# xmlyqing00/V-FloodNet

Hardware: AMD Instinct MI355X
Metric: segmented frames/sec at 480p (higher is better)
Workload: dtype f32

## Files before the change

v-floodnet_amd/csrc/memory_read.hip:

```cpp
#include "common.h"
#include "../../include/vfn_hip.h"
#include <type_traits>
#include <cstdlib>

namespace {

constexpr int DK = 128, DV = 512;
constexpr int CH = 64;

__device__ __forceinline__ int swz(int row, int chunk) { return row * DK + ((chunk ^ (row & 15)) << 2); }

__device__ __forceinline__ int swz64(int row, int chunk) { return row * CH + ((chunk ^ (row & 15)) << 2); }

struct ChunkRegs { f32x4 v[8]; };
__device__ __forceinline__ void chunk_load(ChunkRegs& R, const float* src, int valid, int tid) {
    const int c = tid & 31;
#pragma unroll
    for (int j = 0; j < 8; ++j) {
        const int r = (tid >> 5) + 8 * j;
        const int rr = r < valid ? r : 0;
        R.v[j] = *reinterpret_cast<const f32x4*>(src + (size_t)rr * DK + c * 4);
        if (r >= valid) R.v[j] = f32x4{0.f, 0.f, 0.f, 0.f};
    }
}
// ... 64 lines not shown
        const __bf16 x = (__bf16)a[e], y = (__bf16)b[e];
        h[e] = x; h[4 + e] = y;
        l[e] = (__bf16)(a[e] - (float)x); l[4 + e] = (__bf16)(b[e] - (float)y);
    }
}
__device__ __forceinline__ int swzk(int row, int half, int chunk) { return row * 512 + half * 256 + ((chunk ^ (row & 15)) << 4); }
__device__ __forceinline__ int swzq(int row, int chunk) { return row * 256 + ((chunk ^ (row & 15)) << 4); }

template <int NT, bool X3>
__device__ __forceinline__ void convert_chunk_inplace(float* sK, int tid) {
    constexpr int TPR = NT / CH;
    constexpr int F4 = 32 / TPR;
    const int r = tid / TPR, part = tid % TPR;
    f32x4 v[F4];
#pragma unroll
    for (int j = 0; j < F4; ++j) v[j] = *reinterpret_cast<const f32x4*>(sK + swz(r, part * F4 + j));
    __syncthreads();
    char* base = reinterpret_cast<char*>(sK);
#pragma unroll
    for (int j = 0; j < F4; j += 2) {
        bf16x8 h, l;
        split8(v[j], v[j + 1], h, l);
        const int chunk = (part * F4 + j) >> 1;
        *reinterpret_cast<bf16x8*>(base + swzk(r, 0, chunk)) = h;
        if constexpr (X3) *reinterpret_cast<bf16x8*>(base + swzk(r, 1, chunk)) = l;
    }
    __syncthreads();
}

template <bool X3>
__device__ __forceinline__ void mfma_lp(f32x16& acc, const bf16x8& ah, const bf16x8& al, const bf16x8& bh, const bf16x8& bl) {
    if constexpr (X3) {
        acc = __builtin_amdgcn_mfma_f32_32x32x16_bf16(al, bh, acc, 0, 0, 0);
        acc = __builtin_amdgcn_mfma_f32_32x32x16_bf16(ah, bl, acc, 0, 0, 0);
    }
    acc = __builtin_amdgcn_mfma_f32_32x32x16_bf16(ah, bh, acc, 0, 0, 0);
}

__device__ __forceinline__ float fast_exp(float x) { return __expf(x); }

__device__ __forceinline__ void chunk_range(int B, int nsplit, int split, int& c_lo, int& c_hi) {
    const int nchunks = (B + CH - 1) / CH;
    const int per = (nchunks + nsplit - 1) / nsplit;
    c_lo = split * per;
    c_hi = min(nchunks, c_lo + per);
}

constexpr int QTS = 128;

#ifdef VFN_CENSUS
__device__ unsigned long long vfn_census_buf[4096 * 4];
#endif

struct scan_gather { const int* list; const int* count; };

template <int MODE, int PREC = 0, bool GATHER = false>
__global__ __launch_bounds__(256, 2)
void bank_scan_kernel(const vfn_bankscan_desc p, const scan_gather gather) {
#ifdef VFN_CENSUS
    const unsigned long long census_t0 = __builtin_amdgcn_s_memrealtime();
#endif
    extern __shared__ __attribute__((aligned(16))) char smem[];
    float* sKb = reinterpret_cast<float*>(smem);
    __shared__ int s_item;

    const int tid = threadIdx.x, lane = tid & 63, wave = tid >> 6;
    const int li = lane & 31, lh = lane >> 5;
    const int qtiles = (p.HW + QTS - 1) / QTS;
    int total = p.nsplit * qtiles * p.obj_n;
    if constexpr (GATHER) {
        total = 0;
        for (int o = 0; o < p.obj_n; ++o) total += p.nsplit * ((gather.count[o] + QTS - 1) / QTS);
    }
  for (;;) {
    if (tid == 0) s_item = atomicAdd(p.work_counter, 1);
    __syncthreads();
    int item = s_item;
    __syncthreads();
    if (item >= total) break;
    int obj, qt, split;
    if constexpr (GATHER) {
        obj = 0;
        for (;;) {
            const int n = p.nsplit * ((gather.count[obj] + QTS - 1) / QTS);
            if (item < n) break;
            item -= n; ++obj;
        }
        const int qtl = (gather.count[obj] + QTS - 1) / QTS;
        qt = item % qtl;
        split = item / qtl;
    } else {
        obj = item % p.obj_n;
        qt = (item / p.obj_n) % qtiles;
        split = item / (p.obj_n * qtiles);
    }
    const int q0 = qt * QTS + wave * 32;
    const int ncol = GATHER ? gather.count[obj] : p.HW;
    const int B = p.bank_len[obj];
    const bool lp_image = PREC != 0 && p.bank_k_lp != nullptr;
    const float* K = (lp_image ? reinterpret_cast<const float*>(p.bank_k_lp) : p.bank_k) + (size_t)obj * p.stride_k;
    const float* Q = p.q + (size_t)(p.q_per_obj ? obj : 0) * p.stride_q;

    int c_lo, c_hi;
    chunk_range(B, p.nsplit, split, c_lo, c_hi);
    if (c_lo < c_hi) chunk_load_async(sKb, K + (size_t)c_lo * CH * DK, min(CH, B - c_lo * CH), wave, lane);

    f32x4 qf[PREC == 0 ? 16 : 1];
    bf16x8 qh[PREC == 0 ? 1 : 8], ql[PREC == 2 ? 8 : 1];
    {
        int q = min(q0 + li, ncol - 1);
        if constexpr (GATHER) q = gather.list[(size_t)obj * p.HW + q];
        if constexpr (PREC == 0) {
            const float* qrow = Q + (size_t)q * p.ldq + 4 * lh;
#pragma unroll
            for (int kk = 0; kk < 16; ++kk) qf[kk] = *reinterpret_cast<const f32x4*>(qrow + 8 * kk);
        } else {
            const float* qrow = Q + (size_t)q * p.ldq + 8 * lh;
#pragma unroll
            for (int g = 0; g < 8; ++g) {
                const f32x4 x0 = *reinterpret_cast<const f32x4*>(qrow + 16 * g);
                const f32x4 x1 = *reinterpret_cast<const f32x4*>(qrow + 16 * g + 4);
                if constexpr (PREC == 2) split8(x0, x1, qh[g], ql[g]);
                else qh[g] = cvt8(x0, x1);
            }
        }
    }

    float run_m = -INFINITY, run_l = 0.f;
    int run_i = 0x7fffffff;
    float run_2 = -INFINITY;
    bool sick = false;
    __syncthreads();

    for (int c = c_lo; c < c_hi; ++c) {
        const int b0 = c * CH;
        const float* sK = sKb + ((c - c_lo) & 1) * CH * DK;
#ifndef VFN_ABLATE_KLOAD
        if (c + 1 < c_hi)
            chunk_load_async(sKb + ((c + 1 - c_lo) & 1) * CH * DK, K + (size_t)(b0 + CH) * DK, min(CH, B - b0 - CH), wave, lane);
#endif
        f32x4 scv[MODE >= 1 ? 2 : 1][MODE >= 1 ? 4 : 1];
        float rs_lane = 1.f;
        if constexpr (MODE >= 1) {
            const float* rs = p.rowscale + (size_t)obj * p.stride_rs;
#pragma unroll
            for (int i = 0; i < 2; ++i)
#pragma unroll
                for (int g = 0; g < 4; ++g) scv[i][g] = *reinterpret_cast<const f32x4*>(rs + b0 + 32 * i + 4 * lh + 8 * g);
            if constexpr (MODE == 2) rs_lane = rs[b0 + lane];
        }
// ... 116 lines not shown
                }
            if constexpr (MODE == 2) sick |= (b0 + lane < B) && !(rs_lane > 0.f && rs_lane < 1e12f);
        }
        __syncthreads();
    }

    {
        const float om = __shfl_xor(run_m, 32, 64);
        if (MODE == 0) {
            const float ol = __shfl_xor(run_l, 32, 64);
            const float mn = fmaxf(run_m, om);
            float l = 0.f;
            if (mn > -INFINITY) l = run_l * expf(run_m - mn) + ol * expf(om - mn);
            run_m = mn; run_l = l;
        } else {
            const int oi = __shfl_xor(run_i, 32, 64);
            if constexpr (MODE == 2) {
                const float o2 = __shfl_xor(run_2, 32, 64);
                if (om > run_m || (om == run_m && oi < run_i)) run_2 = fmaxf(run_m, o2);
                else run_2 = fmaxf(run_2, om);
            }
            if (om > run_m || (om == run_m && oi < run_i)) { run_m = om; run_i = oi; }
        }
    }
    if constexpr (MODE == 2) {
        if (__ballot(sick) != 0) run_2 = INFINITY;
    }
#ifdef VFN_CENSUS
    if (threadIdx.x == 0) {
        const int lin = blockIdx.y * gridDim.x + blockIdx.x;
        if (lin < 4096) {
            unsigned hw_id, xcc;
            asm volatile("s_getreg_b32 %0, hwreg(HW_REG_HW_ID)" : "=s"(hw_id));
            asm volatile("s_getreg_b32 %0, hwreg(HW_REG_XCC_ID)" : "=s"(xcc));
            vfn_census_buf[lin * 4] = census_t0; vfn_census_buf[lin * 4 + 1] = __builtin_amdgcn_s_memrealtime();
            vfn_census_buf[lin * 4 + 2] = hw_id; vfn_census_buf[lin * 4 + 3] = xcc;
        }
    }
#endif
    const int q = q0 + li;
    if (lh == 0 && q < ncol) {
        if constexpr (MODE == 2) {
            float* dst = p.part + (((size_t)obj * p.nsplit + split) * p.HW + q) * 4;
            *reinterpret_cast<f32x4*>(dst) = f32x4{run_m, __int_as_float(run_i), run_2, 0.f};
        } else {
            float* dst = p.part + (((size_t)obj * p.nsplit + split) * p.HW + q) * 2;
            dst[0] = run_m;
            dst[1] = (MODE == 0) ? run_l : __int_as_float(run_i);
        }
    }
  }
}

constexpr size_t SCAN_PIPE_LDS = 2 * (size_t)CH * DK * 2 + 2 * CH * sizeof(float);
constexpr unsigned SCAN_PIPE_SC0 = 2 * CH * DK * 2;

template <int MODE>
__global__ __launch_bounds__(256, 2)
void bank_scan_pipe_kernel(const vfn_bankscan_desc p) {
    extern __shared__ __attribute__((aligned(16))) char smem[];
    __shared__ int s_item;

    const int tid = threadIdx.x, lane = tid & 63, wave = tid >> 6;
    const int li = lane & 31, lh = lane >> 5;
    const int qtiles = (p.HW + QTS - 1) / QTS;
    const int total = p.nsplit * qtiles * p.obj_n;
    const int krow = tid >> 2, kc4 = (tid & 3) * 4;
    const unsigned klane_off = (unsigned)krow * 512u + (unsigned)kc4 * 16u;
  for (;;) {
    if (tid == 0) s_item = atomicAdd(p.work_counter, 1);
    __syncthreads();
    const int item = s_item;
    __syncthreads();
    if (item >= total) break;
    const int obj = item % p.obj_n;
    const int qt = (item / p.obj_n) % qtiles;
    const int split = item / (p.obj_n * qtiles);
    const int q0 = qt * QTS + wave * 32;
    const int B = p.bank_len[obj];
    const char* Kimg = reinterpret_cast<const char*>(p.bank_k_lp) + (size_t)obj * p.stride_k * 4;
    const float* Q = p.q + (size_t)(p.q_per_obj ? obj : 0) * p.stride_q;

    int c_lo, c_hi;
    chunk_range(B, p.nsplit, split, c_lo, c_hi);

    u32x4 kst[2][4];
    f32x4 sst[2];
    const float* rs = MODE == 1 ? p.rowscale + (size_t)obj * p.stride_rs : nullptr;
    auto load_k = [&](int c, auto SET_) {
        constexpr int set = decltype(SET_)::value;
        const int b0 = c * CH;
        const __amdgpu_buffer_rsrc_t r = __builtin_amdgcn_make_buffer_rsrc(const_cast<char*>(Kimg + (size_t)b0 * 512), 0, min(CH, B - b0) * 512, 0x00020000);
#pragma unroll
        for (int j = 0; j < 4; ++j) kst[set][j] = __builtin_amdgcn_raw_buffer_load_b128(r, klane_off, 16 * j, 0);
        if constexpr (MODE == 1) { if (tid < 16) sst[set] = *reinterpret_cast<const f32x4*>(rs + b0 + 4 * tid); }
    };
    auto store_k = [&](int buf, auto SET_) {
        constexpr int set = decltype(SET_)::value;
        char* d = smem + buf * (CH * DK * 2);
#pragma unroll
        for (int j = 0; j < 4; ++j) *reinterpret_cast<u32x4*>(d + swzq(krow, kc4 + j)) = kst[set][j];
        if constexpr (MODE == 1) { if (tid < 16) *reinterpret_cast<f32x4*>(smem + SCAN_PIPE_SC0 + buf * (CH * 4) + tid * 16) = sst[set]; }
    };
    using Z0 = std::integral_constant<int, 0>; using Z1 = std::integral_constant<int, 1>;
    if (c_lo < c_hi) load_k(c_lo, Z0{});
    if (c_lo + 1 < c_hi) load_k(c_lo + 1, Z1{});

    bf16x8 qh[8];
    {
        const int q = min(q0 + li, p.HW - 1);
        const float* qrow = Q + (size_t)q * p.ldq + 8 * lh;
#pragma unroll
        for (int g = 0; g < 8; ++g) {
            const f32x4 x0 = *reinterpret_cast<const f32x4*>(qrow + 16 * g);
            const f32x4 x1 = *reinterpret_cast<const f32x4*>(qrow + 16 * g + 4);
            qh[g] = cvt8(x0, x1);
        }
    }

    float run_m = -INFINITY, run_l = 0.f;
    int run_i = 0x7fffffff;
    if (c_lo < c_hi) store_k(0, Z0{});
    __syncthreads();

    auto body = [&](auto PAR_, int c) {
        constexpr int PAR = decltype(PAR_)::value;
        const int b0 = c * CH;
        const char* kb = smem + PAR * (CH * DK * 2);
        if (c + 2 < c_hi) load_k(c + 2, PAR_);
        f32x4 scv[MODE == 1 ? 2 : 1][MODE == 1 ? 4 : 1];
        if constexpr (MODE == 1) {
            const float* sS = reinterpret_cast<const float*>(smem + SCAN_PIPE_SC0 + PAR * (CH * 4));
#pragma unroll
            for (int i = 0; i < 2; ++i)
#pragma unroll
                for (int g = 0; g < 4; ++g) scv[i][g] = *reinterpret_cast<const f32x4*>(sS + 32 * i + 4 * lh + 8 * g);
        }
        f32x16 acc[2];
#pragma unroll
        for (int i = 0; i < 2; ++i)
#pragma unroll
            for (int r = 0; r < 16; ++r) acc[i][r] = 0.f;
#pragma unroll
        for (int g = 0; g < 8; ++g) {
#pragma unroll
            for (int i = 0; i < 2; ++i) {
                const bf16x8 ah = *reinterpret_cast<const bf16x8*>(kb + swzq(32 * i + li, 2 * g + lh));
                acc[i] = __builtin_amdgcn_mfma_f32_32x32x16_bf16(ah, qh[g], acc[i], 0, 0, 0);
            }
        }
        if (MODE == 0) {
            if (b0 + CH <= B) {
                float mx = acc[0][0];
#pragma unroll
                for (int i = 0; i < 2; ++i)
#pragma unroll
                    for (int r = 0; r < 16; ++r) mx = fmaxf(mx, acc[i][r]);
                const float mn = fmaxf(run_m, mx * p.scale);
                float sum = 0.f;
#pragma unroll
                for (int i = 0; i < 2; ++i)
#pragma unroll
                    for (int r = 0; r < 16; ++r) sum += fast_exp(acc[i][r] * p.scale - mn);
                run_l = run_l * expf(run_m - mn) + sum;
                run_m = mn;
            } else {
                float mx = -INFINITY;
#pragma unroll
                for (int i = 0; i < 2; ++i)
#pragma unroll
                    for (int r = 0; r < 16; ++r) {
                        const int row = b0 + 32 * i + 4 * lh + (r & 3) + 8 * (r >> 2);
                        const float s_ = acc[i][r] * p.scale;
                        acc[i][r] = s_;
                        if (row < B) mx = fmaxf(mx, s_);
                    }
                const float mn = fmaxf(run_m, mx);
                if (mn > -INFINITY) {
                    float sum = 0.f;
#pragma unroll
                    for (int i = 0; i < 2; ++i)
#pragma unroll
                        for (int r = 0; r < 16; ++r) {
                            const int row = b0 + 32 * i + 4 * lh + (r & 3) + 8 * (r >> 2);
                            if (row < B) sum += fast_exp(acc[i][r] - mn);
                        }
                    run_l = run_l * expf(run_m - mn) + sum;
                    run_m = mn;
                }
            }
        } else {
#pragma unroll
            for (int i = 0; i < 2; ++i)
#pragma unroll
                for (int g = 0; g < 4; ++g) {
                    const int row0 = b0 + 32 * i + 4 * lh + 8 * g;
                    const f32x4 sc = scv[MODE == 1 ? i : 0][MODE == 1 ? g : 0];
#pragma unroll
                    for (int j = 0; j < 4; ++j) {
                        const int row = row0 + j;
                        if (row < B) {
                            const float s_ = acc[i][4 * g + j] * sc[j];
                            if (s_ > run_m) { run_m = s_; run_i = row; }
                        }
                    }
                }
        }
        if (c + 1 < c_hi) store_k(PAR ^ 1, std::integral_constant<int, PAR ^ 1>{});
        __syncthreads();
    };
    for (int c = c_lo; c < c_hi; c += 2) {
        body(std::integral_constant<int, 0>{}, c);
        if (c + 1 < c_hi) body(std::integral_constant<int, 1>{}, c + 1);
    }

    {
        const float om = __shfl_xor(run_m, 32, 64);
        if (MODE == 0) {
            const float ol = __shfl_xor(run_l, 32, 64);
            const float mn = fmaxf(run_m, om);
            float l = 0.f;
            if (mn > -INFINITY) l = run_l * expf(run_m - mn) + ol * expf(om - mn);
            run_m = mn; run_l = l;
        } else {
            const int oi = __shfl_xor(run_i, 32, 64);
            if (om > run_m || (om == run_m && oi < run_i)) { run_m = om; run_i = oi; }
        }
    }
    const int q = q0 + li;
    if (lh == 0 && q < p.HW) {
        float* dst = p.part + (((size_t)obj * p.nsplit + split) * p.HW + q) * 2;
        dst[0] = run_m;
        dst[1] = (MODE == 0) ? run_l : __int_as_float(run_i);
    }
  }
}

template <int MODE>
__global__ void bank_scan_finish_kernel(const float* __restrict__ part, int nsplit, int HW, int obj_n,
                                        float* __restrict__ ml, int* __restrict__ idx, float* __restrict__ corr,
                                        const float* __restrict__ colscale) {
    const int t = blockIdx.x * blockDim.x + threadIdx.x;
    const int i = min(t >> 3, obj_n * HW - 1), j = t & 7;
    const bool live = (t >> 3) < obj_n * HW;
    const int obj = i / HW, q = i - obj * HW;
    float m = -INFINITY, x = (MODE == 0) ? 0.f : __int_as_float(0x7fffffff);
    auto fold = [&](float om, float ox) {
        if (MODE == 0) {
            const float mn = fmaxf(m, om);
            if (mn > -INFINITY) x = x * expf(m - mn) + ox * expf(om - mn);
            m = mn;
        } else {
            const int i0 = __float_as_int(x), i1 = __float_as_int(ox);
            if (om > m || (om == m && i1 < i0)) { m = om; x = ox; }
        }
    };
    for (int s = j; s < nsplit; s += 8) {
        const float* src = part + (((size_t)obj * nsplit + s) * HW + q) * 2;
        fold(src[0], src[1]);
    }
    const int base = (threadIdx.x & 63) & ~7;
#pragma unroll
    for (int o = 1; o < 8; ++o) {
        const float om = __shfl(m, base + o, 64), ox = __shfl(x, base + o, 64);
        if (j == 0) fold(om, ox);
    }
    if (j != 0 || !live) return;
    if (MODE == 0) { ml[(size_t)i * 2] = m; ml[(size_t)i * 2 + 1] = x; }
    else { idx[i] = __float_as_int(x); corr[i] = m * colscale[i]; }
}

constexpr float MATCH_EPS_REL = 1.25e-4f;
constexpr float MATCH_EPS_ABS = 5.421010862427522e-20f;
constexpr float MATCH_QNORM_MAX = 1.152921504606846976e18f;

__global__ __launch_bounds__(64)
void bank_match_certify_kernel(const vfn_bankmatch_desc p) {
    const int lane = threadIdx.x, li = lane & 31, lh = lane >> 5;
    const int obj = blockIdx.y, q0 = blockIdx.x * 32;
    const int q = q0 + li, qc = min(q, p.HW - 1);
    float m = -INFINITY, m2 = -INFINITY;
    int bi = 0x7fffffff;
    auto fold = [&](float om, int oi, float o2) {
        if (om > m || (om == m && oi < bi)) { m2 = fmaxf(fmaxf(m, m2), o2); m = om; bi = oi; }
        else m2 = fmaxf(fmaxf(m2, om), o2);
    };
    const float* part = p.part_x3 + ((size_t)obj * p.nsplit * p.HW + qc) * 4;
#pragma unroll 4
    for (int s = lh; s < p.nsplit; s += 2) {
        const f32x4 v = *reinterpret_cast<const f32x4*>(part + (size_t)s * p.HW * 4);
        fold(v[0], __float_as_int(v[1]), v[2]);
    }
    fold(__shfl_xor(m, 32, 64), __shfl_xor(bi, 32, 64), __shfl_xor(m2, 32, 64));

    const size_t col = (size_t)obj * p.HW + qc;
    const float qn = p.qnorm[col];
    const float margin = 4.f * (MATCH_EPS_REL * qn + MATCH_EPS_ABS);
    const bool cert = q < p.HW && qn > 0.f && qn <= MATCH_QNORM_MAX && m > -INFINITY && m < INFINITY && (m - m2) > margin;

    const float* krow = p.bank_k + (size_t)obj * p.stride_k + (size_t)(cert ? bi : 0) * DK + 4 * lh;
    const float* qrow = p.q + (size_t)obj * p.stride_q + (size_t)qc * p.ldq + 4 * lh;
    f32x16 acc;
#pragma unroll
    for (int r = 0; r < 16; ++r) acc[r] = 0.f;
#pragma unroll
    for (int kk = 0; kk < 16; ++kk) {
        f32x4 a = *reinterpret_cast<const f32x4*>(krow + 8 * kk);
        const f32x4 b = *reinterpret_cast<const f32x4*>(qrow + 8 * kk);
        if (!cert) a = f32x4{0.f, 0.f, 0.f, 0.f};
#pragma unroll
        for (int t = 0; t < 4; ++t) acc = __builtin_amdgcn_mfma_f32_32x32x2f32(a[t], b[t], acc, 0, 0, 0);
    }
    const int rsel = (li & 3) + 4 * (li >> 3);
    float dot = 0.f;
#pragma unroll
    for (int r = 0; r < 16; ++r) dot = (r == rsel) ? acc[r] : dot;
    if (lh != ((li >> 2) & 1)) return;
    if (cert) {
        const float s_ = dot * p.rowscale[(size_t)obj * p.stride_rs + bi];
        p.match_idx[col] = bi;
        p.match_corr[col] = s_ * p.colscale[col];
    } else if (q < p.HW) {
        const int pos = atomicAdd(p.ucount + obj, 1);
        p.ulist[(size_t)obj * p.HW + pos] = q;
        if (p.utotal) atomicAdd(p.utotal + obj, 1);
    }
}

__global__ void bank_match_finish_listed_kernel(const float* __restrict__ part, int nsplit, int HW, int obj_n,
                                                const int* __restrict__ ulist, const int* __restrict__ ucount,
                                                int* __restrict__ idx, float* __restrict__ corr, const float* __restrict__ colscale) {
    const int t = blockIdx.x * blockDim.x + threadIdx.x;
    const int i = min(t >> 3, obj_n * HW - 1), j = t & 7;
    const int obj = i / HW, pos = i - obj * HW;
    const bool live = (t >> 3) < obj_n * HW && pos < ucount[obj];
    float m = -INFINITY, x = __int_as_float(0x7fffffff);
    auto fold = [&](float om, float ox) {
        const int i0 = __float_as_int(x), i1 = __float_as_int(ox);
        if (om > m || (om == m && i1 < i0)) { m = om; x = ox; }
    };
    if (live)
        for (int s = j; s < nsplit; s += 8) {
            const float* src = part + (((size_t)obj * nsplit + s) * HW + pos) * 2;
            fold(src[0], src[1]);
        }
    const int base = (threadIdx.x & 63) & ~7;
#pragma unroll
    for (int o = 1; o < 8; ++o) {
        const float om = __shfl(m, base + o, 64), ox = __shfl(x, base + o, 64);
        if (j == 0) fold(om, ox);
    }
    if (j != 0 || !live) return;
    const size_t c = (size_t)obj * HW + ulist[(size_t)obj * HW + pos];
    idx[c] = __float_as_int(x);
    corr[c] = m * colscale[c];
}

__device__ __forceinline__ int softmax_hits(f32x16& acc, float scale, float qm, float qinv, float thres, int nvalid, int rloc) {
    int cnt = 0;
#ifdef VFN_ABLATE_SOFTMAX
    for (int r = 0; r < 16; ++r) acc[r] *= qinv;
    return cnt;
#endif
    const float sm = -qm;
    if (nvalid >= CH) {
#pragma unroll
        for (int r = 0; r < 16; ++r) acc[r] = fast_exp(fmaf(acc[r], scale, sm)) * qinv;
    } else {
#pragma unroll
        for (int r = 0; r < 16; ++r) {
            const int rr = rloc + (r & 3) + 8 * (r >> 2);
            const float pv = fast_exp(fmaf(acc[r], scale, sm)) * qinv;
            acc[r] = rr < nvalid ? pv : 0.f;
        }
    }
#pragma unroll
    for (int r = 0; r < 16; ++r) {
        const unsigned long long hit = __ballot(acc[r] > thres);
        const int rlo = (r & 3) + 8 * (r >> 2);
        const int c_lo = __popcll(hit & 0xffffffffull), c_hi = __popcll(hit >> 32);
        asm volatile("v_writelane_b32 %0, %1, %2" : "+v"(cnt) : "s"(c_lo), "n"(rlo));
        asm volatile("v_writelane_b32 %0, %1, %2" : "+v"(cnt) : "s"(c_hi), "n"(rlo + 4));
    }
    return cnt;
}

__device__ int vfn_apply_linear_order = 0;
__device__ __forceinline__ void apply_item(const vfn_memread_desc& p, int& split, int& qt, int& obj) {
    const int qtiles = (int)gridDim.x / p.nsplit;
    if (vfn_apply_linear_order) { split = blockIdx.x % p.nsplit; qt = blockIdx.x / p.nsplit; obj = blockIdx.y; return; }
    const int total = (int)(gridDim.x * gridDim.y);
    const int id = (int)(blockIdx.y * gridDim.x + blockIdx.x);
    const int q = total >> 3, r = total & 7;
    const int xcd = id & 7, slot = id >> 3;
    const int L = (xcd < r ? xcd * (q + 1) : r * (q + 1) + (xcd - r) * q) + slot;
    const int pair = L / qtiles;
    qt = L - pair * qtiles;
    obj = pair / p.nsplit;
    split = pair - obj * p.nsplit;
}

__device__ __forceinline__ int swzp(int row, int chunk) { return row * 128 + ((chunk ^ ((row >> 1) & 7)) << 4); }

constexpr int QTW = 128;

__device__ __forceinline__ void chunk_load_async8(float* sK, const float* src, int valid, int wave, int lane) {
#pragma unroll
    for (int j = 0; j < 4; ++j) {
// ... 853 lines not shown
        f32x4 s = {0.f, 0.f, 0.f, 0.f};
        for (int sp = 0; sp < p.nsplit; ++sp)
            s += *reinterpret_cast<const f32x4*>(p.o_part + (((size_t)obj * p.nsplit + sp) * p.HW + q) * DV + c4 * 4);
        float* o = p.out + ((size_t)obj * p.HW + q) * p.ld_out;
        *reinterpret_cast<f32x4*>(o + c4 * 4) = s;
        if (p.qv) *reinterpret_cast<f32x4*>(o + DV + c4 * 4) = *reinterpret_cast<const f32x4*>(p.qv + (size_t)q * p.ldqv + c4 * 4);
    }
    if (p.cnt) {
        const int B = p.bank_len[obj];
        int* cnt = p.cnt + (size_t)obj * p.stride_cnt;
        float* info = p.info + (size_t)obj * p.stride_info;
        for (int b = blockIdx.x * blockDim.x + threadIdx.x; b < B; b += gridDim.x * blockDim.x) {
            info[(size_t)b * 2 + 1] += logf((float)cnt[b] + 1.f);
            cnt[b] = 0;
        }
    }
}

constexpr size_t SCAN_LDS = (size_t)(2 * CH * DK) * sizeof(float);

bool scores_fit(long long stride_scores, long long stride_k, int HW) {
    const long long cap = stride_k / DK;
    return stride_scores >= ((cap + CH - 1) / CH) * (long long)((HW + 127) / 128) * 8192;
}

template <typename K>
void allow_lds(K kern, size_t bytes) {
    hipFuncSetAttribute(reinterpret_cast<const void*>(kern), hipFuncAttributeMaxDynamicSharedMemorySize, (int)bytes);
}

}

extern "C" int vfn_bank_scan(const vfn_bankscan_desc* d, void* stream) {
    if (!d || !d->q || !d->bank_k || !d->bank_len || !d->part) return VFN_ERR_ARG;
    if (d->nsplit < 1 || d->HW < 1 || d->obj_n < 1 || d->ldq % 4) return VFN_ERR_ARG;
    if (d->mode == 1 && (!d->rowscale || d->stride_rs % 4)) return VFN_ERR_ARG;
    if (d->precision < 0 || d->precision > 2) return VFN_ERR_ARG;
    if (d->scores && (d->mode != 0 || !scores_fit(d->stride_scores, d->stride_k, d->HW))) return VFN_ERR_ARG;
    static bool once = false;
    if (!once) {
        allow_lds(bank_scan_kernel<0, 0>, SCAN_LDS); allow_lds(bank_scan_kernel<1, 0>, SCAN_LDS);
        allow_lds(bank_scan_kernel<0, 1>, SCAN_LDS); allow_lds(bank_scan_kernel<1, 1>, SCAN_LDS);
        allow_lds(bank_scan_kernel<0, 2>, SCAN_LDS); allow_lds(bank_scan_kernel<1, 2>, SCAN_LDS);
        once = true;
    }
    if (!d->work_counter) return VFN_ERR_ARG;
    const int items = cdiv(d->HW, QTS) * d->nsplit * d->obj_n;
    const dim3 grid(items < 512 ? items : 512);
    hipStream_t s = (hipStream_t)stream;
    if (hipMemsetAsync(d->work_counter, 0, sizeof(int), s) != hipSuccess) return VFN_ERR_LAUNCH;
    if (d->precision == 1 && d->bank_k_lp) {
        const char* ep = getenv("VFN_SCAN_PIPE");
        if (!(ep && atoi(ep) == 0)) {
            static int wgs = 0;
            if (!wgs) { const char* ew = getenv("VFN_SCAN_WGS"); wgs = ew ? atoi(ew) : 768; if (wgs < 1) wgs = 768; }
            const dim3 gridp(items < wgs ? items : wgs);
            if (d->mode == 0) hipLaunchKernelGGL((bank_scan_pipe_kernel<0>), gridp, dim3(256), SCAN_PIPE_LDS, s, *d);
            else hipLaunchKernelGGL((bank_scan_pipe_kernel<1>), gridp, dim3(256), SCAN_PIPE_LDS, s, *d);
            return vfn_check_launch();
        }
    }
    switch (d->mode * 3 + d->precision) {
        case 0: hipLaunchKernelGGL((bank_scan_kernel<0, 0>), grid, dim3(256), SCAN_LDS, s, *d, scan_gather{}); break;
        case 1: hipLaunchKernelGGL((bank_scan_kernel<0, 1>), grid, dim3(256), SCAN_LDS, s, *d, scan_gather{}); break;
        case 2: hipLaunchKernelGGL((bank_scan_kernel<0, 2>), grid, dim3(256), SCAN_LDS, s, *d, scan_gather{}); break;
        case 3: hipLaunchKernelGGL((bank_scan_kernel<1, 0>), grid, dim3(256), SCAN_LDS, s, *d, scan_gather{}); break;
        case 4: hipLaunchKernelGGL((bank_scan_kernel<1, 1>), grid, dim3(256), SCAN_LDS, s, *d, scan_gather{}); break;
        case 5: hipLaunchKernelGGL((bank_scan_kernel<1, 2>), grid, dim3(256), SCAN_LDS, s, *d, scan_gather{}); break;
        default: return VFN_ERR_ARG;
    }
    return vfn_check_launch();
}

extern "C" int vfn_bank_scan_finish(const float* part, int nsplit, int HW, int obj_n, int mode, float* ml, int* idx,
                                    float* corr, const float* colscale, void* stream) {
    if (!part) return VFN_ERR_ARG;
    const int total = obj_n * HW;
    if (mode == 0) {
        if (!ml) return VFN_ERR_ARG;
        hipLaunchKernelGGL(bank_scan_finish_kernel<0>, dim3(cdiv(total * 8, 256)), dim3(256), 0, (hipStream_t)stream,
                           part, nsplit, HW, obj_n, ml, idx, corr, colscale);
    } else {
        if (!idx || !corr || !colscale) return VFN_ERR_ARG;
        hipLaunchKernelGGL(bank_scan_finish_kernel<1>, dim3(cdiv(total * 8, 256)), dim3(256), 0, (hipStream_t)stream,
                           part, nsplit, HW, obj_n, ml, idx, corr, colscale);
    }
    return vfn_check_launch();
}

extern "C" int vfn_bank_match_certified(const vfn_bankmatch_desc* d, void* stream) {
    if (!d || !d->q || !d->bank_k || !d->bank_k_lp || !d->bank_len || !d->rowscale || !d->qnorm || !d->colscale) return VFN_ERR_ARG;
    if (!d->part_x3 || !d->part_f32 || !d->ulist || !d->ucount || !d->work_counter || !d->match_idx || !d->match_corr) return VFN_ERR_ARG;
    if (d->nsplit < 1 || d->nsplit_fb < 1 || d->HW < 1 || d->obj_n < 1 || d->ldq % 4 || d->stride_rs % 4) return VFN_ERR_ARG;
    static bool once = false;
    if (!once) {
        allow_lds(bank_scan_kernel<2, 2>, SCAN_LDS); allow_lds(bank_scan_kernel<1, 0, true>, SCAN_LDS);
        once = true;
    }
    hipStream_t s = (hipStream_t)stream;
    vfn_bankscan_desc sd = {};
    sd.q = d->q; sd.bank_k = d->bank_k; sd.bank_len = d->bank_len; sd.rowscale = d->rowscale;
    sd.stride_q = d->stride_q; sd.stride_k = d->stride_k; sd.stride_rs = d->stride_rs;
    sd.scale = 1.f; sd.ldq = d->ldq; sd.q_per_obj = 1; sd.HW = d->HW; sd.obj_n = d->obj_n;
    sd.work_counter = d->work_counter; sd.bank_k_lp = d->bank_k_lp;
    sd.part = d->part_x3; sd.nsplit = d->nsplit; sd.mode = 2; sd.precision = 2;
    const int items = cdiv(d->HW, QTS) * d->nsplit * d->obj_n;
    if (hipMemsetAsync(d->work_counter, 0, sizeof(int), s) != hipSuccess) return VFN_ERR_LAUNCH;
    if (hipMemsetAsync(d->ucount, 0, sizeof(int) * d->obj_n, s) != hipSuccess) return VFN_ERR_LAUNCH;
    hipLaunchKernelGGL((bank_scan_kernel<2, 2>), dim3(items < 512 ? items : 512), dim3(256), SCAN_LDS, s, sd, scan_gather{});
    hipLaunchKernelGGL(bank_match_certify_kernel, dim3(cdiv(d->HW, 32), d->obj_n), dim3(64), 0, s, *d);
    sd.part = d->part_f32; sd.nsplit = d->nsplit_fb; sd.mode = 1; sd.precision = 0; sd.bank_k_lp = nullptr;
    if (hipMemsetAsync(d->work_counter, 0, sizeof(int), s) != hipSuccess) return VFN_ERR_LAUNCH;
    hipLaunchKernelGGL((bank_scan_kernel<1, 0, true>), dim3(512), dim3(256), SCAN_LDS, s, sd, scan_gather{d->ulist, d->ucount});
    hipLaunchKernelGGL(bank_match_finish_listed_kernel, dim3(cdiv(d->obj_n * d->HW * 8, 256)), dim3(256), 0, s,
                       (const float*)d->part_f32, d->nsplit_fb, d->HW, d->obj_n, (const int*)d->ulist, (const int*)d->ucount,
                       d->match_idx, d->match_corr, d->colscale);
    return vfn_check_launch();
}

extern "C" int vfn_memread_apply(const vfn_memread_desc* d, void* stream) {
    if (!d || !d->q || !d->bank_k || !d->bank_v || !d->bank_len || !d->ml || !d->o_part) return VFN_ERR_ARG;
    if (d->nsplit < 1 || d->ldq % 4) return VFN_ERR_ARG;
    if (d->precision < 0 || d->precision > 2) return VFN_ERR_ARG;
    if (d->scores && !scores_fit(d->stride_scores, d->stride_k, d->HW)) return VFN_ERR_ARG;
    {
        static bool once_x = false;
        if (!once_x) {
            const char* e = getenv("VFN_APPLY_XCD");
            const int lin = (e && atoi(e) == 0) ? 1 : 0;
            if (lin && hipMemcpyToSymbol(HIP_SYMBOL(vfn_apply_linear_order), &lin, sizeof(int)) != hipSuccess) return VFN_ERR_LAUNCH;
            once_x = true;
        }
    }
    if (d->precision == 0) {
        static bool once_f = false;
        constexpr size_t LDS_WF = (size_t)(QTW * DK + CH * DK + QTW * CH) * sizeof(float);
        if (!once_f) { allow_lds(memread_apply_wide_kernel, LDS_WF); once_f = true; }
        const dim3 gridw(cdiv(d->HW, QTW) * d->nsplit, d->obj_n);
        if (d->scores) hipLaunchKernelGGL(memread_apply_ss_kernel, gridw, dim3(512), (size_t)2 * QTW * CH * sizeof(float), (hipStream_t)stream, *d);
        else hipLaunchKernelGGL(memread_apply_wide_kernel, gridw, dim3(512), LDS_WF, (hipStream_t)stream, *d);
        return vfn_check_launch();
    }
    {
        static bool once_w = false;
        constexpr size_t LDS_W1 = (size_t)QTW * DK * 2 + (size_t)CH * DK * 4 + 2 * (size_t)QTW * CH * 2;
        constexpr size_t LDS_W2 = LDS_W1 + (size_t)QTW * DK * 2;
        if (!once_w) { allow_lds(memread_apply_lpw_kernel<false>, LDS_W1); allow_lds(memread_apply_lpw_kernel<true>, LDS_W2); once_w = true; }
        const dim3 gridw(cdiv(d->HW, QTW) * d->nsplit, d->obj_n);
        static int img_bf16 = 1;
        if (d->bank_k_lp && d->bank_v_lp && (d->precision == 2 || img_bf16)) {
            static bool once_s = false;
            if (!once_s) {
                allow_lds(memread_apply_shw_kernel<true>, LDS_W2);
                allow_lds(memread_apply_shw_kernel<false>, LDS_W1);
                const char* e = getenv("VFN_APPLY_IMG_BF16");
                if (e) img_bf16 = atoi(e);
                once_s = true;
            }
            static bool once_p = false;
            if (!once_p) { allow_lds(memread_apply_pipe_kernel, APPLY_PIPE_LDS); once_p = true; }
            const char* ep = getenv("VFN_APPLY_PIPE");
            const bool pipe = !(ep && atoi(ep) == 0);
            if (d->precision == 2) hipLaunchKernelGGL(memread_apply_shw_kernel<true>, gridw, dim3(512), LDS_W2, (hipStream_t)stream, *d);
            else if (img_bf16 && pipe) hipLaunchKernelGGL(memread_apply_pipe_kernel, gridw, dim3(512), APPLY_PIPE_LDS, (hipStream_t)stream, *d);
            else if (img_bf16) hipLaunchKernelGGL(memread_apply_shw_kernel<false>, gridw, dim3(512), LDS_W1, (hipStream_t)stream, *d);
            if (d->precision == 2 || img_bf16) return vfn_check_launch();
        }
        if (d->precision == 1) hipLaunchKernelGGL(memread_apply_lpw_kernel<false>, gridw, dim3(512), LDS_W1, (hipStream_t)stream, *d);
        else hipLaunchKernelGGL(memread_apply_lpw_kernel<true>, gridw, dim3(512), LDS_W2, (hipStream_t)stream, *d);
// ... 19 lines not shown
```

Before: 160.6.

## Add top-k certification, self-resetting work counters, and optional x3 pipelined scan

The certified bank-match path gets a new top-k certify kernel, enabled by default. It collects up to eight near-best candidates per column from the split partials and re-scores them exactly in f32 with MFMA, so fewer columns fall back to the full f32 gather scan. The scan kernels now reset the work counter on the last draw, and a single-block gather_finish kernel resets ucount, which removes the per-call hipMemsetAsync operations. An optional pipelined x3 (hi/lo bf16) scan variant is added behind an environment variable. The single-block finish kernel may serialise work when many columns are uncertified.

```diff
diff --git a/v-floodnet_amd/csrc/memory_read.hip b/v-floodnet_amd/csrc/memory_read.hip
--- a/v-floodnet_amd/csrc/memory_read.hip
+++ b/v-floodnet_amd/csrc/memory_read.hip
@@ -140,7 +140,41 @@
 __device__ unsigned long long vfn_census_buf[4096 * 4];
 #endif
 
-struct scan_gather { const int* list; const int* count; };
+struct scan_gather { const int* list; int* count; int* idx; float* corr; const float* colscale; };
+
+__device__ __forceinline__ bool last_draw(int item, int total) { return item == total + (int)gridDim.x - 1; }
+__device__ __forceinline__ int gcount(const scan_gather& g, int obj, int HW) { return min(g.count[obj], HW); }
+
+__device__ void gather_finish(const vfn_bankscan_desc& p, const scan_gather& g, int tid) {
+    int ncol = 0;
+    for (int o = 0; o < p.obj_n; ++o) ncol += gcount(g, o, p.HW);
+    const int lane = tid & 63, wave = tid >> 6;
+    for (int c = wave; c < ncol; c += 4) {
+        int i = c, obj = 0;
+        while (i >= gcount(g, obj, p.HW)) { i -= gcount(g, obj, p.HW); ++obj; }
+        float m = -INFINITY, x = __int_as_float(0x7fffffff);
+        auto fold = [&](float om, float ox) {
+            const int i0 = __float_as_int(x), i1 = __float_as_int(ox);
+            if (om > m || (om == m && i1 < i0)) { m = om; x = ox; }
+        };
+        for (int s = lane; s < p.nsplit; s += 64) {
+            const float* src = p.part + (((size_t)obj * p.nsplit + s) * p.HW + i) * 2;
+            fold(src[0], src[1]);
+        }
+#pragma unroll
+        for (int o = 32; o >= 1; o >>= 1) fold(__shfl_xor(m, o, 64), __shfl_xor(x, o, 64));
+        if (lane == 0) {
+            const size_t cc = (size_t)obj * p.HW + g.list[(size_t)obj * p.HW + i];
+            g.idx[cc] = __float_as_int(x);
+            g.corr[cc] = m * g.colscale[cc];
+        }
+    }
+    __syncthreads();
+    for (int o = tid; o < p.obj_n; o += 256) atomicExch(g.count + o, 0);
+}
+
+__global__ __launch_bounds__(256)
+void gather_finish_kernel(const vfn_bankscan_desc p, const scan_gather g) { gather_finish(p, g, threadIdx.x); }
 
 template <int MODE, int PREC = 0, bool GATHER = false>
 __global__ __launch_bounds__(256, 2)
@@ -158,23 +192,26 @@
     int total = p.nsplit * qtiles * p.obj_n;
     if constexpr (GATHER) {
         total = 0;
-        for (int o = 0; o < p.obj_n; ++o) total += p.nsplit * ((gather.count[o] + QTS - 1) / QTS);
+        for (int o = 0; o < p.obj_n; ++o) total += p.nsplit * ((gcount(gather, o, p.HW) + QTS - 1) / QTS);
     }
   for (;;) {
     if (tid == 0) s_item = atomicAdd(p.work_counter, 1);
     __syncthreads();
     int item = s_item;
     __syncthreads();
-    if (item >= total) break;
+    if (item >= total) {
+        if (tid == 0 && last_draw(item, total)) atomicExch(p.work_counter, 0);
+        break;
+    }
     int obj, qt, split;
     if constexpr (GATHER) {
         obj = 0;
         for (;;) {
-            const int n = p.nsplit * ((gather.count[obj] + QTS - 1) / QTS);
+            const int n = p.nsplit * ((gcount(gather, obj, p.HW) + QTS - 1) / QTS);
             if (item < n) break;
             item -= n; ++obj;
         }
-        const int qtl = (gather.count[obj] + QTS - 1) / QTS;
+        const int qtl = (gcount(gather, obj, p.HW) + QTS - 1) / QTS;
         qt = item % qtl;
         split = item / qtl;
     } else {
@@ -183,7 +220,7 @@
         split = item / (p.obj_n * qtiles);
     }
     const int q0 = qt * QTS + wave * 32;
-    const int ncol = GATHER ? gather.count[obj] : p.HW;
+    const int ncol = GATHER ? gcount(gather, obj, p.HW) : p.HW;
     const int B = p.bank_len[obj];
     const bool lp_image = PREC != 0 && p.bank_k_lp != nullptr;
     const float* K = (lp_image ? reinterpret_cast<const float*>(p.bank_k_lp) : p.bank_k) + (size_t)obj * p.stride_k;
@@ -406,27 +443,35 @@
   }
 }
 
-constexpr size_t SCAN_PIPE_LDS = 2 * (size_t)CH * DK * 2 + 2 * CH * sizeof(float);
-constexpr unsigned SCAN_PIPE_SC0 = 2 * CH * DK * 2;
+template <int MODE> constexpr unsigned scan_pipe_row() { return MODE == 2 ? 512u : 256u; }
+template <int MODE> constexpr unsigned scan_pipe_sc0() { return 2 * CH * scan_pipe_row<MODE>(); }
+template <int MODE> constexpr size_t scan_pipe_lds() { return scan_pipe_sc0<MODE>() + 2 * CH * sizeof(float); }
+constexpr size_t SCAN_PIPE_LDS = scan_pipe_lds<0>();
 
 template <int MODE>
 __global__ __launch_bounds__(256, 2)
 void bank_scan_pipe_kernel(const vfn_bankscan_desc p) {
     extern __shared__ __attribute__((aligned(16))) char smem[];
     __shared__ int s_item;
+    constexpr bool X3 = MODE == 2;
+    constexpr unsigned ROWB = scan_pipe_row<MODE>(), SC0 = scan_pipe_sc0<MODE>();
+    constexpr int KJ = X3 ? 8 : 4;
 
     const int tid = threadIdx.x, lane = tid & 63, wave = tid >> 6;
     const int li = lane & 31, lh = lane >> 5;
     const int qtiles = (p.HW + QTS - 1) / QTS;
     const int total = p.nsplit * qtiles * p.obj_n;
-    const int krow = tid >> 2, kc4 = (tid & 3) * 4;
+    const int krow = tid >> 2, kc4 = (tid & 3) * KJ;
     const unsigned klane_off = (unsigned)krow * 512u + (unsigned)kc4 * 16u;
   for (;;) {
     if (tid == 0) s_item = atomicAdd(p.work_counter, 1);
     __syncthreads();
     const int item = s_item;
     __syncthreads();
-    if (item >= total) break;
+    if (item >= total) {
+        if (tid == 0 && last_draw(item, total)) atomicExch(p.work_counter, 0);
+        break;
+    }
     const int obj = item % p.obj_n;
     const int qt = (item / p.obj_n) % qtiles;
     const int split = item / (p.obj_n * qtiles);
@@ -438,29 +483,32 @@
     int c_lo, c_hi;
     chunk_range(B, p.nsplit, split, c_lo, c_hi);
 
-    u32x4 kst[2][4];
+    u32x4 kst[2][KJ];
     f32x4 sst[2];
-    const float* rs = MODE == 1 ? p.rowscale + (size_t)obj * p.stride_rs : nullptr;
+    const float* rs = MODE >= 1 ? p.rowscale + (size_t)obj * p.stride_rs : nullptr;
     auto load_k = [&](int c, auto SET_) {
         constexpr int set = decltype(SET_)::value;
         const int b0 = c * CH;
         const __amdgpu_buffer_rsrc_t r = __builtin_amdgcn_make_buffer_rsrc(const_cast<char*>(Kimg + (size_t)b0 * 512), 0, min(CH, B - b0) * 512, 0x00020000);
 #pragma unroll
-        for (int j = 0; j < 4; ++j) kst[set][j] = __builtin_amdgcn_raw_buffer_load_b128(r, klane_off, 16 * j, 0);
-        if constexpr (MODE == 1) { if (tid < 16) sst[set] = *reinterpret_cast<const f32x4*>(rs + b0 + 4 * tid); }
+        for (int j = 0; j < KJ; ++j) kst[set][j] = __builtin_amdgcn_raw_buffer_load_b128(r, klane_off, 16 * j, 0);
+        if constexpr (MODE >= 1) { if (tid < 16) sst[set] = *reinterpret_cast<const f32x4*>(rs + b0 + 4 * tid); }
     };
     auto store_k = [&](int buf, auto SET_) {
         constexpr int set = decltype(SET_)::value;
-        char* d = smem + buf * (CH * DK * 2);
-#pragma unroll
-        for (int j = 0; j < 4; ++j) *reinterpret_cast<u32x4*>(d + swzq(krow, kc4 + j)) = kst[set][j];
-        if constexpr (MODE == 1) { if (tid < 16) *reinterpret_cast<f32x4*>(smem + SCAN_PIPE_SC0 + buf * (CH * 4) + tid * 16) = sst[set]; }
+        char* d = smem + buf * (CH * ROWB);
+#pragma unroll
+        for (int j = 0; j < KJ; ++j) {
+            const int cc = kc4 + j;
+            *reinterpret_cast<u32x4*>(d + (X3 ? swzk(krow, cc >> 4, cc & 15) : swzq(krow, cc))) = kst[set][j];
+        }
+        if constexpr (MODE >= 1) { if (tid < 16) *reinterpret_cast<f32x4*>(smem + SC0 + buf * (CH * 4) + tid * 16) = sst[set]; }
     };
     using Z0 = std::integral_constant<int, 0>; using Z1 = std::integral_constant<int, 1>;
     if (c_lo < c_hi) load_k(c_lo, Z0{});
     if (c_lo + 1 < c_hi) load_k(c_lo + 1, Z1{});
 
-    bf16x8 qh[8];
+    bf16x8 qh[8], ql[X3 ? 8 : 1];
     {
         const int q = min(q0 + li, p.HW - 1);
         const float* qrow = Q + (size_t)q * p.ldq + 8 * lh;
@@ -468,23 +516,26 @@
         for (int g = 0; g < 8; ++g) {
             const f32x4 x0 = *reinterpret_cast<const f32x4*>(qrow + 16 * g);
             const f32x4 x1 = *reinterpret_cast<const f32x4*>(qrow + 16 * g + 4);
-            qh[g] = cvt8(x0, x1);
+            if constexpr (X3) split8(x0, x1, qh[g], ql[g]);
+            else qh[g] = cvt8(x0, x1);
         }
     }
 
     float run_m = -INFINITY, run_l = 0.f;
     int run_i = 0x7fffffff;
+    float run_2 = -INFINITY;
+    bool sick = false;
     if (c_lo < c_hi) store_k(0, Z0{});
     __syncthreads();
 
     auto body = [&](auto PAR_, int c) {
         constexpr int PAR = decltype(PAR_)::value;
         const int b0 = c * CH;
-        const char* kb = smem + PAR * (CH * DK * 2);
+        const char* kb = smem + PAR * (CH * ROWB);
         if (c + 2 < c_hi) load_k(c + 2, PAR_);
         f32x4 scv[MODE == 1 ? 2 : 1][MODE == 1 ? 4 : 1];
+        const float* sS = reinterpret_cast<const float*>(smem + SC0 + PAR * (CH * 4));
         if constexpr (MODE == 1) {
-            const float* sS = reinterpret_cast<const float*>(smem + SCAN_PIPE_SC0 + PAR * (CH * 4));
 #pragma unroll
             for (int i = 0; i < 2; ++i)
 #pragma unroll
@@ -499,8 +550,14 @@
         for (int g = 0; g < 8; ++g) {
 #pragma unroll
             for (int i = 0; i < 2; ++i) {
-                const bf16x8 ah = *reinterpret_cast<const bf16x8*>(kb + swzq(32 * i + li, 2 * g + lh));
-                acc[i] = __builtin_amdgcn_mfma_f32_32x32x16_bf16(ah, qh[g], acc[i], 0, 0, 0);
+                if constexpr (X3) {
+                    const bf16x8 ah = *reinterpret_cast<const bf16x8*>(kb + swzk(32 * i + li, 0, 2 * g + lh));
+                    const bf16x8 al = *reinterpret_cast<const bf16x8*>(kb + swzk(32 * i + li, 1, 2 * g + lh));
+                    mfma_lp<true>(acc[i], ah, al, qh[g], ql[g]);
+                } else {
+                    const bf16x8 ah = *reinterpret_cast<const bf16x8*>(kb + swzq(32 * i + li, 2 * g + lh));
+                    acc[i] = __builtin_amdgcn_mfma_f32_32x32x16_bf16(ah, qh[g], acc[i], 0, 0, 0);
+                }
             }
         }
         if (MODE == 0) {
@@ -549,16 +606,22 @@
 #pragma unroll
                 for (int g = 0; g < 4; ++g) {
                     const int row0 = b0 + 32 * i + 4 * lh + 8 * g;
-                    const f32x4 sc = scv[MODE == 1 ? i : 0][MODE == 1 ? g : 0];
+                    const f32x4 sc = MODE == 2 ? *reinterpret_cast<const f32x4*>(sS + 32 * i + 4 * lh + 8 * g)
+                                               : scv[MODE == 1 ? i : 0][MODE == 1 ? g : 0];
 #pragma unroll
                     for (int j = 0; j < 4; ++j) {
                         const int row = row0 + j;
                         if (row < B) {
                             const float s_ = acc[i][4 * g + j] * sc[j];
+                            if constexpr (MODE == 2) run_2 = __builtin_amdgcn_fmed3f(s_, run_m, run_2);
                             if (s_ > run_m) { run_m = s_; run_i = row; }
                         }
                     }
                 }
+            if constexpr (MODE == 2) {
+                const float rs_lane = sS[lane];
+                sick |= (b0 + lane < B) && !(rs_lane > 0.f && rs_lane < 1e12f);
+            }
         }
         if (c + 1 < c_hi) store_k(PAR ^ 1, std::integral_constant<int, PAR ^ 1>{});
         __syncthreads();
@@ -578,14 +641,27 @@
             run_m = mn; run_l = l;
         } else {
             const int oi = __shfl_xor(run_i, 32, 64);
+            if constexpr (MODE == 2) {
+                const float o2 = __shfl_xor(run_2, 32, 64);
+                if (om > run_m || (om == run_m && oi < run_i)) run_2 = fmaxf(run_m, o2);
+                else run_2 = fmaxf(run_2, om);
+            }
             if (om > run_m || (om == run_m && oi < run_i)) { run_m = om; run_i = oi; }
         }
+    }
+    if constexpr (MODE == 2) {
+        if (__ballot(sick) != 0) run_2 = INFINITY;
     }
     const int q = q0 + li;
     if (lh == 0 && q < p.HW) {
-        float* dst = p.part + (((size_t)obj * p.nsplit + split) * p.HW + q) * 2;
-        dst[0] = run_m;
-        dst[1] = (MODE == 0) ? run_l : __int_as_float(run_i);
+        if constexpr (MODE == 2) {
+            float* dst = p.part + (((size_t)obj * p.nsplit + split) * p.HW + q) * 4;
+            *reinterpret_cast<f32x4*>(dst) = f32x4{run_m, __int_as_float(run_i), run_2, 0.f};
+        } else {
+            float* dst = p.part + (((size_t)obj * p.nsplit + split) * p.HW + q) * 2;
+            dst[0] = run_m;
+            dst[1] = (MODE == 0) ? run_l : __int_as_float(run_i);
+        }
     }
   }
 }
@@ -676,38 +752,109 @@
         p.match_corr[col] = s_ * p.colscale[col];
     } else if (q < p.HW) {
         const int pos = atomicAdd(p.ucount + obj, 1);
-        p.ulist[(size_t)obj * p.HW + pos] = q;
+        if (pos < p.HW) p.ulist[(size_t)obj * p.HW + pos] = q;
         if (p.utotal) atomicAdd(p.utotal + obj, 1);
     }
 }
 
-__global__ void bank_match_finish_listed_kernel(const float* __restrict__ part, int nsplit, int HW, int obj_n,
-                                                const int* __restrict__ ulist, const int* __restrict__ ucount,
-                                                int* __restrict__ idx, float* __restrict__ corr, const float* __restrict__ colscale) {
-    const int t = blockIdx.x * blockDim.x + threadIdx.x;
-    const int i = min(t >> 3, obj_n * HW - 1), j = t & 7;
-    const int obj = i / HW, pos = i - obj * HW;
-    const bool live = (t >> 3) < obj_n * HW && pos < ucount[obj];
-    float m = -INFINITY, x = __int_as_float(0x7fffffff);
-    auto fold = [&](float om, float ox) {
-        const int i0 = __float_as_int(x), i1 = __float_as_int(ox);
-        if (om > m || (om == m && i1 < i0)) { m = om; x = ox; }
-    };
-    if (live)
-        for (int s = j; s < nsplit; s += 8) {
-            const float* src = part + (((size_t)obj * nsplit + s) * HW + pos) * 2;
-            fold(src[0], src[1]);
-        }
-    const int base = (threadIdx.x & 63) & ~7;
+constexpr int MATCH_KMAX = 8;
+__global__ __launch_bounds__(256)
+void bank_match_certify_topk_kernel(const vfn_bankmatch_desc p) {
+    __shared__ int s_cnt[32], s_off[33], s_cand[32][MATCH_KMAX];
+    __shared__ int s_pb[32 * MATCH_KMAX], s_pc[32 * MATCH_KMAX];
+    __shared__ float s_pf[32 * MATCH_KMAX];
+    const int tid = threadIdx.x, lane = tid & 63, wave = tid >> 6, li = lane & 31, lh = lane >> 5;
+    const int obj = blockIdx.y, q0 = blockIdx.x * 32;
+    const int cl = tid >> 3, j = tid & 7, gbase = lane & ~7;
+    const int q = q0 + cl, qc = min(q, p.HW - 1);
+    if (tid < 32) s_cnt[tid] = 0;
+
+    const float* part = p.part_x3 + ((size_t)obj * p.nsplit * p.HW + qc) * 4;
+    float a1 = -INFINITY, R = -INFINITY;
+    for (int s = j; s < p.nsplit; s += 8) {
+        const f32x4 v = *reinterpret_cast<const f32x4*>(part + (size_t)s * p.HW * 4);
+        a1 = fmaxf(a1, v[0]); R = fmaxf(R, v[2]);
+    }
 #pragma unroll
     for (int o = 1; o < 8; ++o) {
-        const float om = __shfl(m, base + o, 64), ox = __shfl(x, base + o, 64);
-        if (j == 0) fold(om, ox);
-    }
-    if (j != 0 || !live) return;
-    const size_t c = (size_t)obj * HW + ulist[(size_t)obj * HW + pos];
-    idx[c] = __float_as_int(x);
-    corr[c] = m * colscale[c];
+        const float oa = __shfl(a1, gbase + o, 64), orr = __shfl(R, gbase + o, 64);
+        if (j == 0) { a1 = fmaxf(a1, oa); R = fmaxf(R, orr); }
+    }
+    a1 = __shfl(a1, gbase, 64); R = __shfl(R, gbase, 64);
+    const size_t col = (size_t)obj * p.HW + qc;
+    const float qn = p.qnorm[col];
+    const float margin = 4.f * (MATCH_EPS_REL * qn + MATCH_EPS_ABS);
+    bool cert = q < p.HW && qn > 0.f && qn <= MATCH_QNORM_MAX && a1 > -INFINITY && a1 < INFINITY && (a1 - R) > margin;
+    __syncthreads();
+
+    if (cert)
+        for (int s = j; s < p.nsplit; s += 8) {
+            const f32x4 v = *reinterpret_cast<const f32x4*>(part + (size_t)s * p.HW * 4);
+            if (a1 - v[0] <= margin) {
+                const int pos = atomicAdd(&s_cnt[cl], 1);
+                if (pos < MATCH_KMAX) s_cand[cl][pos] = __float_as_int(v[1]);
+            }
+        }
+    __syncthreads();
+    if (tid == 0) {
+        int o = 0;
+        for (int c = 0; c < 32; ++c) { s_off[c] = o; const int n = s_cnt[c]; o += n <= MATCH_KMAX ? n : 0; }
+        s_off[32] = o;
+    }
+    __syncthreads();
+    if (j < MATCH_KMAX && j < s_cnt[cl] && s_cnt[cl] <= MATCH_KMAX) {
+        s_pb[s_off[cl] + j] = s_cand[cl][j];
+        s_pc[s_off[cl] + j] = qc;
+    }
+    __syncthreads();
+
+    const int npairs = s_off[32];
+    for (int b0 = 32 * wave; b0 < npairs; b0 += 128) {
+        const int pi = b0 + li;
+        const bool pl = pi < npairs;
+        const int eb = pl ? s_pb[pi] : 0, pq = pl ? s_pc[pi] : qc;
+        const float* krow = p.bank_k + (size_t)obj * p.stride_k + (size_t)eb * DK + 4 * lh;
+        const float* qrow = p.q + (size_t)obj * p.stride_q + (size_t)pq * p.ldq + 4 * lh;
+        f32x16 acc;
+#pragma unroll
+        for (int r = 0; r < 16; ++r) acc[r] = 0.f;
+#pragma unroll
+        for (int kk = 0; kk < 16; ++kk) {
+            f32x4 a = *reinterpret_cast<const f32x4*>(krow + 8 * kk);
+            const f32x4 b = *reinterpret_cast<const f32x4*>(qrow + 8 * kk);
+            if (!pl) a = f32x4{0.f, 0.f, 0.f, 0.f};
+#pragma unroll
+            for (int t = 0; t < 4; ++t) acc = __builtin_amdgcn_mfma_f32_32x32x2f32(a[t], b[t], acc, 0, 0, 0);
+        }
+        const int rsel = (li & 3) + 4 * (li >> 3);
+        float dot = 0.f;
+#pragma unroll
+        for (int r = 0; r < 16; ++r) dot = (r == rsel) ? acc[r] : dot;
+        if (pl && lh == ((li >> 2) & 1)) s_pf[pi] = dot * p.rowscale[(size_t)obj * p.stride_rs + eb];
+    }
+    __syncthreads();
+
+    if (j != 0) return;
+    const int n = s_cnt[cl];
+    cert = cert && n <= MATCH_KMAX;
+    float m = -INFINITY;
+    int bi = 0x7fffffff;
+    if (cert) {
+        for (int k = 0; k < n; ++k) {
+            const float f = s_pf[s_off[cl] + k];
+            const int b = s_pb[s_off[cl] + k];
+            if (f > m || (f == m && b < bi)) { m = f; bi = b; }
+        }
+        cert = m > -INFINITY && m < INFINITY;
+    }
+    if (cert) {
+        p.match_idx[col] = bi;
+        p.match_corr[col] = m * p.colscale[col];
+    } else if (q < p.HW) {
+        const int pos = atomicAdd(p.ucount + obj, 1);
+        if (pos < p.HW) p.ulist[(size_t)obj * p.HW + pos] = q;
+        if (p.utotal) atomicAdd(p.utotal + obj, 1);
+    }
 }
 
 __device__ __forceinline__ int softmax_hits(f32x16& acc, float scale, float qm, float qinv, float thres, int nvalid, int rloc) {
@@ -1667,6 +1814,7 @@
     if (d->precision == 1 && d->bank_k_lp) {
         const char* ep = getenv("VFN_SCAN_PIPE");
         if (!(ep && atoi(ep) == 0)) {
+            if ((d->mode != 0 && d->mode != 1) || d->scores) return VFN_ERR_ARG;
             static int wgs = 0;
             if (!wgs) { const char* ew = getenv("VFN_SCAN_WGS"); wgs = ew ? atoi(ew) : 768; if (wgs < 1) wgs = 768; }
             const dim3 gridp(items < wgs ? items : wgs);
@@ -1710,8 +1858,13 @@
     static bool once = false;
     if (!once) {
         allow_lds(bank_scan_kernel<2, 2>, SCAN_LDS); allow_lds(bank_scan_kernel<1, 0, true>, SCAN_LDS);
+        allow_lds(bank_scan_pipe_kernel<2>, scan_pipe_lds<2>());
         once = true;
     }
+    const char* ep = getenv("VFN_SCAN_X3_PIPE");
+    const bool pipe = ep && atoi(ep) == 1;
+    const char* et = getenv("VFN_MATCH_TOPK");
+    const bool topk = !(et && atoi(et) == 0);
     hipStream_t s = (hipStream_t)stream;
     vfn_bankscan_desc sd = {};
     sd.q = d->q; sd.bank_k = d->bank_k; sd.bank_len = d->bank_len; sd.rowscale = d->rowscale;
@@ -1720,16 +1873,19 @@
     sd.work_counter = d->work_counter; sd.bank_k_lp = d->bank_k_lp;
     sd.part = d->part_x3; sd.nsplit = d->nsplit; sd.mode = 2; sd.precision = 2;
     const int items = cdiv(d->HW, QTS) * d->nsplit * d->obj_n;
-    if (hipMemsetAsync(d->work_counter, 0, sizeof(int), s) != hipSuccess) return VFN_ERR_LAUNCH;
-    if (hipMemsetAsync(d->ucount, 0, sizeof(int) * d->obj_n, s) != hipSuccess) return VFN_ERR_LAUNCH;
-    hipLaunchKernelGGL((bank_scan_kernel<2, 2>), dim3(items < 512 ? items : 512), dim3(256), SCAN_LDS, s, sd, scan_gather{});
-    hipLaunchKernelGGL(bank_match_certify_kernel, dim3(cdiv(d->HW, 32), d->obj_n), dim3(64), 0, s, *d);
+    if (pipe) {
+        static int wgs = 0;
+        if (!wgs) { const char* ew = getenv("VFN_SCAN_X3_WGS"); wgs = ew ? atoi(ew) : 512; if (wgs < 1) wgs = 512; }
+        hipLaunchKernelGGL((bank_scan_pipe_kernel<2>), dim3(items < wgs ? items : wgs), dim3(256), scan_pipe_lds<2>(), s, sd);
+    } else {
+        hipLaunchKernelGGL((bank_scan_kernel<2, 2>), dim3(items < 512 ? items : 512), dim3(256), SCAN_LDS, s, sd, scan_gather{});
+    }
+    if (topk) hipLaunchKernelGGL(bank_match_certify_topk_kernel, dim3(cdiv(d->HW, 32), d->obj_n), dim3(256), 0, s, *d);
+    else hipLaunchKernelGGL(bank_match_certify_kernel, dim3(cdiv(d->HW, 32), d->obj_n), dim3(64), 0, s, *d);
     sd.part = d->part_f32; sd.nsplit = d->nsplit_fb; sd.mode = 1; sd.precision = 0; sd.bank_k_lp = nullptr;
-    if (hipMemsetAsync(d->work_counter, 0, sizeof(int), s) != hipSuccess) return VFN_ERR_LAUNCH;
-    hipLaunchKernelGGL((bank_scan_kernel<1, 0, true>), dim3(512), dim3(256), SCAN_LDS, s, sd, scan_gather{d->ulist, d->ucount});
-    hipLaunchKernelGGL(bank_match_finish_listed_kernel, dim3(cdiv(d->obj_n * d->HW * 8, 256)), dim3(256), 0, s,
-                       (const float*)d->part_f32, d->nsplit_fb, d->HW, d->obj_n, (const int*)d->ulist, (const int*)d->ucount,
-                       d->match_idx, d->match_corr, d->colscale);
+    const scan_gather sg{d->ulist, d->ucount, d->match_idx, d->match_corr, d->colscale};
+    hipLaunchKernelGGL((bank_scan_kernel<1, 0, true>), dim3(512), dim3(256), SCAN_LDS, s, sd, sg);
+    hipLaunchKernelGGL(gather_finish_kernel, dim3(1), dim3(256), 0, s, sd, sg);
     return vfn_check_launch();
 }
 
```

Result: no change. 161.5 (median of 6 runs) (+0.6%).
